# lifthrasiir/j40

Measured on AMD Instinct MI355X. Metric: Mpixels/s RGBA-u8x4 decode, 8K VarDCT d1, higher is better.
Workload: dtype f32

## Files before the change

### j40_amd/csrc/device/hf_lanes_dev.h

```cpp
#pragma once
#include "hf_dev.h"

namespace j40hip {

struct LaneTables {
	const J40_LDS uint8_t *ctx_map;
	const J40_LDS uint32_t *cluster_cfg;
	const J40_LDS uint64_t *alias;
	const J40_LDS int16_t *nnz_ctx2;
	const J40_LDS int8_t *freq_ctx2;
	const J40_LDS uint32_t *dct_info;
	int32_t log_alpha, log_bucket;
};

struct LaneFrame {
	int32_t nb_block_ctx, num_hf_presets, preset_bits, check_section_end;
	uint32_t single_declared_end;
	const J40_GLOBAL uint32_t *order_off;
};

struct LaneGlobals {
	const J40_GLOBAL uint8_t *codestream;
	const J40_GLOBAL uint32_t *group_blocks;
	J40_GLOBAL float *coeffs;
	J40_GLOBAL CoeffEvent *events;
	J40_GLOBAL uint32_t *block_events;
	const J40_GLOBAL uint16_t *pool_u16;
	uint32_t coeff_stride;
};

struct LaneBits {
	const J40_GLOBAL uint8_t *base;
	uint64_t bits;
	int32_t nbits;
	uint32_t pos;
	uint32_t ahead;
};

J40_DEV uint32_t lane_load32(const J40_GLOBAL uint8_t *base, uint32_t pos) { return *(const J40_GLOBAL uint32_t *) (base + pos); }

J40_DEV void lane_bits_init(LaneBits &b, const J40_GLOBAL uint8_t *base, uint32_t start_bit) {
	b.base = base;
	const uint32_t pos0 = (start_bit >> 3) & ~3u, skip = start_bit - 8u * pos0;
	b.bits = (uint64_t) (lane_load32(base, pos0) >> skip);
	b.nbits = 32 - (int32_t) skip;
	b.pos = pos0 + 4;
	b.ahead = lane_load32(base, b.pos);
}

J40_DEV void lane_bits_refill(LaneBits &b) {
	if (b.nbits <= 32) {
		b.bits |= (uint64_t) b.ahead << b.nbits;
		b.nbits += 32;
		b.pos += 4u;
		b.ahead = lane_load32(b.base, b.pos);
	}
}

J40_DEV uint32_t lane_bits_take(LaneBits &b, int32_t n) {
	const uint32_t v = (uint32_t) b.bits & ((1u << n) - 1u);
	b.bits >>= n; b.nbits -= n;
	return v;
}

J40_DEV uint32_t lane_bit_position(const LaneBits &b) { return 8u * b.pos - (uint32_t) b.nbits; }

template <bool STRAIGHT = false, bool STARTED = false, class AliasPtr>
J40_DEV int32_t lane_symbol_in_cluster(LaneBits &b, uint32_t &state, AliasPtr alias, int32_t log_alpha, int32_t log_bucket, uint32_t cl, uint32_t m, uint32_t end_bit, uint32_t *err) {
	if (!STRAIGHT && !STARTED && state == 0) {
		state = lane_bits_take(b, 16); state |= lane_bits_take(b, 16) << 16;
		lane_bits_refill(b);
	}
	const uint32_t idx = state & 0xfff, i = idx >> log_bucket, pos = idx & ((1u << log_bucket) - 1);
	const uint64_t e = alias[(cl << log_alpha) + i];
	const uint32_t elo = (uint32_t) e, ehi = (uint32_t) (e >> 32);
	const bool aliased = pos >= (elo & 0xff);
	const int32_t token = (int32_t) (aliased ? (elo >> 20) & 0xff : i);
	const uint32_t offset = aliased ? (elo >> 8) & 0xfff : 0;
	const uint32_t d = aliased ? (uint32_t) (e >> 28) & 0x1fff : (ehi >> 9) & 0x1fff;
	state = d * (state >> 12) + offset + pos;
	const bool renorm = state < (1u << 16);
	const uint32_t low = lane_bits_take(b, renorm ? 16 : 0);
	state = renorm ? (state << 16) | low : state;
	const bool short1 = lane_bit_position(b) > end_bit;
	const int32_t split_exp = (int32_t) (m & 15), split = 1 << split_exp;
	const bool big = token >= split;
	const int32_t mt = (int32_t) (m >> 12);
	const bool iovf = big && token > mt;
	const int32_t tok = iovf ? mt : token;
	const int32_t msb = (int32_t) ((m >> 4) & 15), lsb = (int32_t) ((m >> 8) & 15), in_token = msb + lsb;
	const int32_t midbits = big ? split_exp - in_token + ((tok - split) >> in_token) : 0;
	if (!STRAIGHT && midbits > b.nbits) lane_bits_refill(b);
	const int32_t mid = (int32_t) lane_bits_take(b, midbits);
	const bool short2 = lane_bit_position(b) > end_bit;
	const int32_t top = 1 << msb;
	const int32_t lo = tok & ((1 << lsb) - 1), hi = (tok >> lsb) & (top - 1);
	const int32_t value = ((top | hi) << (midbits + lsb)) | ((mid << lsb) | lo);
	*err = short1 ? (uint32_t) ERR_SHRT : iovf ? (uint32_t) ERR_IOVF : short2 ? (uint32_t) ERR_SHRT : 0u;
	return big ? value : token;
}
template <class Tables>
J40_DEV int32_t lane_symbol(LaneBits &b, uint32_t &state, const Tables &t, int32_t ctx, uint32_t end_bit, uint32_t *err) {
	const uint32_t cl = t.ctx_map[ctx];
	return lane_symbol_in_cluster(b, state, t.alias, t.log_alpha, t.log_bucket, cl, t.cluster_cfg[cl], end_bit, err);
}

typedef uint32_t LaneEventQuad __attribute__((vector_size(16)));

J40_DEV void lane_store_block_events(const LaneGlobals &G, uint32_t blk, uint32_t first, uint32_t n0, uint32_t n1, uint32_t n2) {
	J40_GLOBAL uint64_t *e = (J40_GLOBAL uint64_t *) (G.block_events + 4u * blk);
	e[0] = (uint64_t) first | ((uint64_t) n0 << 32); e[1] = (uint64_t) n1 | ((uint64_t) n2 << 32);
}

struct LaneSection {
	uint32_t start_bit, end_bit;
	uint32_t cell_base;
	uint32_t block_first; int32_t nblocks;
	uint32_t ev_first, ev_end;
};

#ifndef J40_LANE_NZ_PERIOD
#define J40_LANE_NZ_PERIOD 8
#endif
#ifndef J40_LANE_STRAIGHT_COEFFS
#define J40_LANE_STRAIGHT_COEFFS 1
#endif
#ifndef J40_LANE_REFILL_SELECTS
#define J40_LANE_REFILL_SELECTS 0
#endif
template <bool SCAN, class Source>
J40_DEV void decode_hf_sections_lane(const LaneFrame &f, const LaneTables &t, const LaneGlobals &G, Source &src, J40_LDS int8_t *cols, int32_t col_stride, int32_t pass, J40_LDS uint32_t *ring = nullptr, int32_t ring_stride = 0) {
	LaneSection S;
	S.start_bit = S.end_bit = S.cell_base = S.block_first = S.ev_first = S.ev_end = 0; S.nblocks = 0;
	LaneBits b;
	b.base = G.codestream; b.bits = 0; b.nbits = 0; b.pos = 0; b.ahead = 0;
	const int32_t nb_block_ctx = f.nb_block_ctx;
	uint32_t err = 0, end_bit = 0, cell64 = 0, block_first = 0;
	int32_t nblocks = 0, ctxoff = 0;
	bool have = false;
	int32_t k = 0, c_yxb = 0;
	bool in_coeffs = false, done = true;
	uint32_t state = 0;
	int32_t x8 = 0, y8 = 0, log_columns = 3, order_idx = 0, shift = 0, size = 64;
	uint32_t coeffoff = 0, coeff_at = 0, bctx3 = 0;
	int32_t c = 1, bctx = 0, nz = 0, i = 0, prev = 0, cctx = 0;
	const J40_GLOBAL uint16_t *order = nullptr;
	uint32_t ev_at = 0, ev_end = 0, chan_first = 0;
	uint32_t ev_flushed = 0;
	uint32_t blk_first = 0, blk_n0 = 0, blk_n1 = 0;
	uint32_t next0 = 0, next1 = 0;
	for (uint32_t turn = 0; ; ++turn) {
#if J40_LANE_EV_FLUSH
		if (SCAN && (turn % J40_LANE_EV_FLUSH) == 0) {
#ifdef __HIPCC__
			asm volatile("");
#endif
			if (ev_at - ev_flushed >= (uint32_t) J40_LANE_EV_FLUSH) {
			const J40_LDS uint32_t *r = ring + (int32_t) (ev_flushed % (uint32_t) HF_LANE_RING_SLOTS) * ring_stride;
			J40_GLOBAL uint32_t *dst = (J40_GLOBAL uint32_t *) G.events + ev_flushed;
#pragma unroll
			for (int32_t k4 = 0; k4 < J40_LANE_EV_FLUSH; k4 += 4) {
				LaneEventQuad q4;
				q4[0] = r[k4 * ring_stride]; q4[1] = r[(k4 + 1) * ring_stride]; q4[2] = r[(k4 + 2) * ring_stride]; q4[3] = r[(k4 + 3) * ring_stride];
				*(J40_GLOBAL LaneEventQuad *) (dst + k4) = q4;
			}
			ev_flushed += (uint32_t) J40_LANE_EV_FLUSH;
			}
		}
#endif
		if (SCAN && J40_LANE_STRAIGHT_COEFFS) {
			if (in_coeffs && !done && state != 0) {
				if (J40_LANE_REFILL_SELECTS) {
					const bool need = b.nbits <= 32;
					b.bits |= (uint64_t) (need ? b.ahead : 0u) << (need ? b.nbits : 0);
					b.nbits += need ? 32 : 0; b.pos += need ? 4u : 0u;
					b.ahead = lane_load32(b.base, b.pos);
				} else lane_bits_refill(b);
				const int32_t cctx_now = cctx + t.nnz_ctx2[(nz + (1 << shift) - 1) >> shift] + t.freq_ctx2[i >> shift] + prev;
				uint32_t e2;
				const uint32_t cl = t.ctx_map[cctx_now];
				const int32_t v = lane_symbol_in_cluster<false, true>(b, state, t.alias, t.log_alpha, t.log_bucket, cl, t.cluster_cfg[cl], end_bit, &e2);
				const bool nonzero = v != 0 && e2 == 0;
				const int32_t sv = unpack_signed_dev(v);
				const bool full = nonzero && (ev_at >= ev_end || !coeff_event_fits(sv));
				if (nonzero && !full) {
					if (J40_LANE_EV_FLUSH) ring[(int32_t) (ev_at % (uint32_t) HF_LANE_RING_SLOTS) * ring_stride] = coeff_event_pack((uint32_t) i, sv);
					else ((J40_GLOBAL uint32_t *) G.events)[ev_at] = coeff_event_pack((uint32_t) i, sv);
				}
				ev_at += nonzero && !full ? 1u : 0u;
				e2 = e2 ? e2 : full ? (uint32_t) ERR_EVOF : 0u;
				prev = v != 0;
				nz -= prev;
				++i;
				in_coeffs = nz != 0;
				e2 = e2 ? e2 : in_coeffs && i >= size ? (uint32_t) ERR_COEF : 0u;
				const bool next_channel = !in_coeffs && e2 == 0;
				c_yxb += next_channel ? 1 : 0;
				const bool next_block = next_channel && c_yxb == 3;
				c_yxb = next_block ? 0 : c_yxb;
				k += next_block ? 1 : 0;
				err = e2 ? e2 : err;
				done = e2 != 0 || (next_block && k >= nblocks);
			}
			if ((turn % J40_LANE_NZ_PERIOD) != 0) continue;
#ifdef __HIPCC__
			asm volatile("");
#endif
			if (in_coeffs && !done && state != 0) continue;
		}
		if (done) {
			if (have) {
				if (SCAN && J40_LANE_EV_FLUSH) for (; ev_flushed < ev_at; ++ev_flushed) ((J40_GLOBAL uint32_t *) G.events)[ev_flushed] = ring[(int32_t) (ev_flushed % (uint32_t) HF_LANE_RING_SLOTS) * ring_stride];
				if (SCAN && !err && nblocks > 0) lane_store_block_events(G, block_first + (uint32_t) nblocks - 1u, blk_first, blk_n0, blk_n1, ev_at - chan_first);
				if (!err) {
					if (state == 0) { lane_bits_refill(b); state = lane_bits_take(b, 16); state |= lane_bits_take(b, 16) << 16; if (lane_bit_position(b) > end_bit) err = ERR_SHRT; }
					if (!err && state != 0x130000) err = ERR_ANS;
				}
				if (!err && f.check_section_end) {
					const uint32_t at = lane_bit_position(b), padn = (0u - at) & 7u;
					if (padn > (uint32_t) b.nbits) lane_bits_refill(b);
					if (lane_bits_take(b, (int32_t) padn)) err = ERR_PAD0;
					else if (at + padn != 8u * f.single_declared_end) err = at + padn < 8u * f.single_declared_end ? (uint32_t) ERR_SHRT : (uint32_t) ERR_EXCS;
				}
				src.done(err, lane_bit_position(b));
			}
			have = src.next(S);
			if (!have) break;
			end_bit = S.end_bit; cell64 = S.cell_base * 64u; block_first = S.block_first; nblocks = S.nblocks;
			lane_bits_init(b, G.codestream, S.start_bit);
			lane_bits_refill(b);
			err = 0;
			const uint32_t preset = lane_bits_take(b, f.preset_bits);
			if (lane_bit_position(b) > end_bit) err = ERR_SHRT;
			else if ((int32_t) preset >= f.num_hf_presets) err = ERR_RNGE;
			ctxoff = 495 * nb_block_ctx * (int32_t) preset;
			k = 0; c_yxb = 0; in_coeffs = false; state = 0;
			ev_at = chan_first = blk_first = ev_flushed = S.ev_first; ev_end = S.ev_end; blk_n0 = blk_n1 = 0;
			done = nblocks == 0 || err != 0;
			if (done) continue;
			{ const J40_GLOBAL uint32_t *p = G.group_blocks + 2u * block_first; next0 = p[0]; next1 = p[1]; }
		}
		if (!in_coeffs && (turn % J40_LANE_NZ_PERIOD) != 0) continue;
		lane_bits_refill(b);
		int32_t ctx;
		if (!in_coeffs) {
			if (SCAN) {
				const uint32_t n = ev_at - chan_first;
				if (c_yxb == 1) blk_n0 = n; else if (c_yxb == 2) blk_n1 = n;
				else if (k > 0) lane_store_block_events(G, block_first + (uint32_t) k - 1u, blk_first, blk_n0, blk_n1, n);
				chan_first = ev_at;
			}
			if (c_yxb == 0) {
				const uint32_t w = next1;
				coeffoff = next0 & ~15u;
				blk_first = ev_at;
				if (k + 1 < nblocks) { const J40_GLOBAL uint32_t *p = G.group_blocks + 2u * (block_first + (uint32_t) k + 1u); next0 = p[0]; next1 = p[1]; }
				x8 = (int32_t) (w & 31); y8 = (int32_t) ((w >> 5) & 31); bctx3 = w >> 16;
				const uint32_t di = t.dct_info[(w >> 10) & 31];
				log_columns = (int32_t) ((di >> 8) & 255); order_idx = (int32_t) (di >> 16);
				shift = (int32_t) (di & 255) + log_columns - 6; size = 64 << shift;
			}
			c = c_yxb == 0 ? 1 : c_yxb == 1 ? 0 : 2;
			bctx = (int32_t) ((bctx3 >> (4 * c_yxb)) & 15);
			const J40_LDS int8_t *col = cols + (c * 32 + x8) * col_stride;
			const int32_t left = x8 > 0 ? col[-col_stride] : -1, topv = y8 > 0 ? col[0] : -1;
			const int32_t pnz = left < 0 ? (topv < 0 ? 32 : topv) : topv < 0 ? left : (left + topv + 1) >> 1;
			ctx = ctxoff + bctx + (pnz < 8 ? pnz : 4 + pnz / 2) * nb_block_ctx;
		} else {
			ctx = cctx + t.nnz_ctx2[(nz + (1 << shift) - 1) >> shift] + t.freq_ctx2[i >> shift] + prev;
		}
		uint32_t e2;
		const int32_t v = lane_symbol(b, state, t, ctx, end_bit, &e2);
		if (!in_coeffs) {
			nz = v;
			e2 = e2 ? e2 : nz > (63 << shift) ? (uint32_t) ERR_COEF : 0u;
			const int8_t qnz = (int8_t) ((nz + (1 << shift) - 1) >> shift);
			J40_LDS int8_t *col = cols + (c * 32 + x8) * col_stride;
			for (int32_t q = 0; q < (1 << (log_columns - 3)); ++q) col[q * col_stride] = qnz;
			cctx = ctxoff + 458 * bctx + 37 * nb_block_ctx;
			prev = nz <= (size >> 4);
			i = 1 << shift;
			if (!SCAN) {
				coeff_at = (uint32_t) c * G.coeff_stride + cell64 + coeffoff;
				order = G.pool_u16 + f.order_off[(pass * 13 + order_idx) * 3 + c];
			}
			in_coeffs = nz > 0;
		} else {
			const bool nonzero = v != 0 && e2 == 0;
			if (SCAN) {
// ... 46 lines not shown
```

### j40_amd/csrc/device/kernels.hip

```cpp
#include <hip/hip_runtime.h>
#include <hip/hip_ext.h>
#include <type_traits>
#include <cstring>
#include <cstdlib>
#include "hf_dev.h"
#include "hf_lanes_dev.h"
#include "idct_dev.h"
#include "vardct_dev.h"
#include "special8_dev.h"
#include "large_dev.h"
#include "k2_iter_dev.h"
#include "hf_uni_dev.h"
#include "restore_dev.h"
#include "kernels.h"

namespace j40hip {

__constant__ float c_half_secants[256];
__constant__ float c_afv_basis[256];
__device__ float c_srgb_thr[SRGB_TABLE_FLOATS];

#define J40_STAGE_SRGB_THRESHOLDS(f) \
	__shared__ float s_srgb_thr[SRGB_TABLE_FLOATS]; \
	for (int32_t i_ = threadIdx.x; i_ < SRGB_TABLE_FLOATS; i_ += blockDim.x) s_srgb_thr[i_] = c_srgb_thr[i_]; \
// ... 241 lines not shown
	const J40_GLOBAL DevPlan &plan = ((const J40_GLOBAL DevPlan *) plans)[w.frame];
	const J40_GLOBAL DevFrame &df = *(const J40_GLOBAL DevFrame *) plan.frame;
	const bool active = lane < w.num_groups;
	auto align16 = [](uint32_t v) { return (v + 15u) & ~15u; };
	LaneFrame f;
	f.nb_block_ctx = df.nb_block_ctx; f.num_hf_presets = df.num_hf_presets; f.preset_bits = df.preset_bits; f.check_section_end = df.check_section_end; f.single_declared_end = df.single_declared_end;
	f.order_off = df.order_off;
	const int32_t num_passes = df.num_passes, num_groups = df.num_groups, scan = df.sparse_coeffs;
	LaneGlobals G;
	G.codestream = (const J40_GLOBAL uint8_t *) plan.codestream;
	G.group_blocks = (const J40_GLOBAL uint32_t *) plan.group_blocks;
	G.coeffs = (J40_GLOBAL float *) plan.coeffs[0];
	G.events = (J40_GLOBAL CoeffEvent *) plan.events; G.block_events = (J40_GLOBAL uint32_t *) plan.block_events;
	G.pool_u16 = (const J40_GLOBAL uint16_t *) plan.pool_u16;
	G.coeff_stride = plan.coeff_stride;
	const J40_GLOBAL uint8_t *pool_u8 = (const J40_GLOBAL uint8_t *) plan.pool_u8;
	const J40_GLOBAL int32_t *pool_i32 = (const J40_GLOBAL int32_t *) plan.pool_i32;
	const J40_GLOBAL uint64_t *pool_u64 = (const J40_GLOBAL uint64_t *) plan.pool_u64;
	const J40_GLOBAL DevCodeSpec *specs = (const J40_GLOBAL DevCodeSpec *) plan.coeff_specs;
	const J40_GLOBAL DevCluster *clusters = (const J40_GLOBAL DevCluster *) plan.clusters;
	LaneQueue q;
	q.sections = (const J40_GLOBAL DevSection *) plan.sections; q.lf_groups = (const J40_GLOBAL DevLfGroup *) plan.lf_groups;
	q.block_start = (const J40_GLOBAL uint32_t *) plan.group_block_start; q.ev_range = (const J40_GLOBAL uint32_t *) plan.ev_range;
	q.lane_order = (const J40_GLOBAL uint32_t *) plan.lane_order;
	q.status = (J40_GLOBAL uint32_t *) plan.status; q.end_bits = df.sections_have_trailer ? (J40_GLOBAL uint32_t *) plan.section_end_bit : nullptr;
	q.counter = w.pad && queue && num_passes == 1 ? (J40_GLOBAL uint32_t *) queue + w.frame : nullptr;
	q.num_groups = num_groups; q.scan = scan != 0; q.g = 0;

	J40_LDS uint8_t *lds = (J40_LDS uint8_t *) hf_lds;
	J40_LDS int16_t *l_nnz = (J40_LDS int16_t *) lds;
	J40_LDS int8_t *l_freq = (J40_LDS int8_t *) (lds + 128);
	J40_LDS uint32_t *l_dct = (J40_LDS uint32_t *) (lds + 192);
	const uint32_t off_pass = 192 + 112;
	if (tid < 64) { l_nnz[tid] = DEV_NNZ_CTX2[tid]; l_freq[tid] = DEV_FREQ_CTX2[tid]; }
	if (tid < 27) l_dct[tid] = (uint32_t) DEV_DCT_SELECT[tid][0] | ((uint32_t) DEV_DCT_SELECT[tid][1] << 8) | ((uint32_t) DEV_DCT_SELECT[tid][2] << 16);
	LaneTables t;
	t.nnz_ctx2 = l_nnz; t.freq_ctx2 = l_freq; t.dct_info = l_dct;
	J40_LDS int8_t *l_cols = (J40_LDS int8_t *) (lds + lds_tables_bytes + (uint32_t) (tid >> 6) * HF_LANE_COLS_BYTES) + lane;
	J40_LDS uint32_t *l_ring = (J40_LDS uint32_t *) (lds + lds_tables_bytes + (uint32_t) (tid >> 6) * HF_LANE_COLS_BYTES + HF_LANE_PRED_BYTES) + lane;
	for (int32_t pass = 0; pass < num_passes; ++pass) {
		const J40_GLOBAL DevCodeSpec &spec = specs[pass];
		__syncthreads();
		const int32_t num_dist = spec.num_dist, num_clusters = spec.num_clusters, log_alpha = spec.log_alpha_size;
		J40_LDS uint8_t *l_map = lds + off_pass;
		J40_LDS uint32_t *l_cfg = (J40_LDS uint32_t *) (lds + off_pass + align16((uint32_t) num_dist));
		J40_LDS uint64_t *l_alias = (J40_LDS uint64_t *) ((J40_LDS uint8_t *) l_cfg + align16(4u * (uint32_t) num_clusters));
		{
			const J40_GLOBAL uint32_t *msrc = (const J40_GLOBAL uint32_t *) (pool_u8 + spec.cluster_map_off);
			J40_LDS uint32_t *mdst = (J40_LDS uint32_t *) l_map;
			for (int32_t i = tid; i < (num_dist + 3) / 4; i += blockDim.x) mdst[i] = msrc[i];
			const J40_GLOBAL int32_t *csrc = pool_i32 + spec.lane_cfg_off;
			for (int32_t i = tid; i < num_clusters; i += blockDim.x) l_cfg[i] = (uint32_t) csrc[i];
			const J40_GLOBAL uint64_t *asrc = pool_u64 + clusters[spec.cluster_off].table_off;
			for (uint32_t i = tid; i < ((uint32_t) num_clusters << log_alpha); i += blockDim.x) l_alias[i] = asrc[i];
		}
		t.ctx_map = l_map; t.cluster_cfg = l_cfg; t.alias = l_alias; t.log_alpha = log_alpha; t.log_bucket = 12 - log_alpha;
		__syncthreads();
		q.pass = pass; q.slot = active ? w.first_group + lane : -1;
		if (scan) decode_hf_sections_lane<true>(f, t, G, q, l_cols, 64, pass, l_ring, 64);
		else decode_hf_sections_lane<false>(f, t, G, q, l_cols, 64, pass);
	}
}

void launch_hf_lanes(const DevPlan *plans, const HfLaneWork *work, int32_t num_work, int32_t waves_per_wg, uint32_t lds_bytes, hipStream_t stream, hipEvent_t started, hipEvent_t stopped, uint32_t *queue) {
	if (num_work <= 0) return;
	static bool configured = false;
	if (!configured) { (void) hipFuncSetAttribute((const void *) k_hf_lanes, hipFuncAttributeMaxDynamicSharedMemorySize, 160 * 1024); configured = true; }
	const uint32_t tables = (lds_bytes + 15u) & ~15u;
	if (started && stopped) hipExtLaunchKernelGGL(k_hf_lanes, dim3((unsigned) (num_work / waves_per_wg)), dim3(64u * (unsigned) waves_per_wg), tables + (uint32_t) waves_per_wg * HF_LANE_COLS_BYTES, stream, started, stopped, 0, plans, work, tables, queue);
	else hipLaunchKernelGGL(k_hf_lanes, dim3((unsigned) (num_work / waves_per_wg)), dim3(64u * (unsigned) waves_per_wg), tables + (uint32_t) waves_per_wg * HF_LANE_COLS_BYTES, stream, plans, work, tables, queue);
}

uint32_t hf_lanes_lds_bytes(const HfLaunchInfo &info) {
	auto align16 = [](uint32_t v) { return (v + 15u) & ~15u; };
	uint32_t n = align16(info.block_ctx_size) + 192;
	if (info.tables_fit_lds) n += align16(info.max_num_dist) + align16(info.max_clusters * (uint32_t) sizeof(DevCluster)) + align16(info.max_table_bytes);
	return n;
}

void launch_hf_entropy_lanes(const DevPlan *plans, const HfLaneWork *work, int32_t num_work, bool tables_in_lds, uint32_t lds_bytes, hipStream_t stream) {
	if (num_work <= 0) return;
	if (tables_in_lds) {
		static bool configured = false;
		if (!configured) { (void) hipFuncSetAttribute((const void *) k_hf_entropy_lanes<true>, hipFuncAttributeMaxDynamicSharedMemorySize, 160 * 1024); configured = true; }
		hipLaunchKernelGGL(k_hf_entropy_lanes<true>, dim3((unsigned) num_work), dim3(64), lds_bytes, stream, plans, work);
	} else {
		hipLaunchKernelGGL(k_hf_entropy_lanes<false>, dim3((unsigned) num_work), dim3(64), lds_bytes, stream, plans, work);
	}
}


#ifdef J40_K2_PHASES
__device__ unsigned long long g_k2_phase[64][8];
#define K2_PHASES_BEGIN unsigned long long k2_acc[8] = {0, 0, 0, 0, 0, 0, 0, 0}; unsigned long long k2_last = __builtin_amdgcn_s_memtime()
#define K2_PHASE(i) do { const unsigned long long now_ = __builtin_amdgcn_s_memtime(); k2_acc[i] += now_ - k2_last; k2_last = now_; } while (0)
#define K2_PHASES_END(slot) do { if (threadIdx.x == 0) for (int i_ = 0; i_ < 8; ++i_) atomicAdd(&g_k2_phase[slot][i_], k2_acc[i_]); } while (0)
extern "C" __attribute__((visibility("default"))) void j40hip_debug_k2_phases(unsigned long long *out, int reset) {
	(void) hipDeviceSynchronize();
	(void) hipMemcpyFromSymbol(out, HIP_SYMBOL(g_k2_phase), sizeof(unsigned long long) * 64 * 8, 0, hipMemcpyDeviceToHost);
	if (reset) { static unsigned long long zero[64 * 8]; (void) hipMemcpyToSymbol(HIP_SYMBOL(g_k2_phase), zero, sizeof zero, 0, hipMemcpyHostToDevice); }
}
#else
#define K2_PHASES_BEGIN do { } while (0)
#define K2_PHASE(i) do { } while (0)
#define K2_PHASES_END(slot) do { } while (0)
#endif

__device__ __forceinline__ void uniform_plan(DevPlan &p) {
	p.frame = uni(p.frame); p.pool_u16 = uni(p.pool_u16); p.pool_f32 = uni(p.pool_f32); p.events = uni(p.events); p.block_events = uni(p.block_events);
	for (int c = 0; c < 3; ++c) { p.llf[c] = uni(p.llf[c]); p.coeffs[c] = uni(p.coeffs[c]); }
	p.coeff_stride = uni(p.coeff_stride);
}
// ... 776 lines not shown
```

### j40_amd/csrc/device/lf_rows_dev.h

```cpp
#pragma once
#include "lf_lanes_dev.h"
#include "modular_dev.h"

namespace j40hip {

enum { LF_USES_RAW = 1u << 8 };
J40_DEV uint32_t lf_stopped_at(int32_t chan, int32_t done) { return ((uint32_t) chan << 24) | (uint32_t) done; }

enum { LF_ROW_WIN = 256,
       LF_ROW_PITCH = LF_ROW_WIN + 2 };

struct LfRowTables {
	const J40_LDS DevTreeNode *tree;
	const J40_LDS uint32_t *fast;
	const J40_GLOBAL uint64_t *alias;
	int32_t log_alpha, log_bucket;
	uint32_t uses;
};

typedef uint32_t LfFastQuad __attribute__((vector_size(16)));
enum { LF_FAST_IOVF = 1u << 18, LF_FAST_IOVF_BASE = 1u << 30 };
J40_DEV void lf_rows_token_info(uint32_t tok, uint32_t cfg, uint32_t *base, uint32_t *extra, uint32_t *iovf) {
	const uint32_t split_exp = cfg & 15u, split = 1u << split_exp, msb = (cfg >> 4) & 15u, lsb = (cfg >> 8) & 15u, in_token = msb + lsb, mt = cfg >> 12;
	*base = tok; *extra = 0; *iovf = 0;
// ... 265 lines not shown
		return;
	}
	L.flush_n = ((cw - 1) & (LF_ROW_WIN - 1)) + 1; L.flush_dst = L.row + (cw - L.flush_n);
	L.x = 0; L.y = y + 1; L.row += cw; L.pw = L.pww = 0; L.a0 = L.a1 = 0;
	if (L.y < L.chh) {
		if (wide) { L.a2 = L.row[-cw]; L.a3 = L.row[1 - cw]; L.a4 = L.row[2 - cw]; }
		else { L.a2 = L.win[0]; L.a3 = cw > 1 ? L.win[1] : 0; L.a4 = cw > 2 ? L.win[2] : 0; }
		return;
	}
	++L.chan; L.setup = true;
}

J40_DEV int32_t lf_row_plain_run(const LfRowLane &L) {
	const bool can = L.plain_ok & !L.setup & (L.chan < 7) & (L.state != 0) & (!L.plain_wide | (L.x > 0));
	const int32_t last = L.plain_wide ? mod_min(L.cw - 1, L.x | (LF_ROW_WIN - 1)) : L.cw - 1;
	return can ? mod_max(last + 1 - L.x, 0) : 0;
}
J40_DEV void lf_row_run_end(LfRowLane &L) {
	if (lf_row_deferred(L)) return;
	const int32_t cw = L.cw, nx = L.x;
	if (nx < cw) {
		L.flush_n = LF_ROW_WIN; L.flush_dst = L.row + (nx - LF_ROW_WIN);
		return;
	}
	L.flush_n = ((cw - 1) & (LF_ROW_WIN - 1)) + 1; L.flush_dst = L.row + (cw - L.flush_n);
	L.x = 0; L.y += 1; L.row += cw; L.pw = L.pww = 0; L.a0 = L.a1 = 0;
	if (L.y < L.chh) {
		if (cw > LF_ROW_WIN) { L.a2 = L.row[-cw]; L.a3 = L.row[1 - cw]; L.a4 = L.row[2 - cw]; }
		else { L.a2 = L.win[0]; L.a3 = cw > 1 ? L.win[1] : 0; L.a4 = cw > 2 ? L.win[2] : 0; }
		return;
	}
	++L.chan; L.setup = true;
}
J40_DEV void lf_row_step(LfRowLane &L, const J40_GLOBAL DevLfTask &t, const LfRowTables &T) {
	if (L.in_run) lf_row_run_end(L); else lf_row_step_general(L, t, T);
	L.plain_left = lf_row_plain_run(L);
	L.in_run = L.plain_left > 0;
	L.live = !lf_row_done(L);
}

#ifdef __HIPCC__
J40_DEV int32_t lf_mad24(int32_t a, int32_t b, int32_t c) { int32_t d; asm("v_mad_i32_i24 %0, %1, %2, %3" : "=v"(d) : "v"(a), "v"(b), "v"(c)); return d; }
#else
J40_DEV int32_t lf_mad24(int32_t a, int32_t b, int32_t c) { return a * b + c; }
#endif
J40_DEV int32_t lf_unzigzag(int32_t u) { return (int32_t) ((uint32_t) u >> 1) ^ -(u & 1); }

enum { LF_NEED_TEST = 1,
       LF_NEED_LIN = 2, LF_NEED_SEL = 4, LF_NEED_GRAD = 8,
       LF_NEED_MUL = 16,
       LF_NEED_ALL = 31,
       LF_NEED_PRED = LF_NEED_TEST | LF_NEED_LIN | LF_NEED_SEL | LF_NEED_GRAD };

#ifdef __HIPCC__
J40_DEV uint32_t lf_bfe(uint32_t v, uint32_t off, uint32_t width) { return __builtin_amdgcn_ubfe(v, off, width); }
J40_DEV uint32_t lf_renorm_word(uint32_t state, uint32_t window) { return __builtin_amdgcn_perm(state, window, 0x05040100u); }
#else
J40_DEV uint32_t lf_bfe(uint32_t v, uint32_t off, uint32_t width) { return width ? (v >> off) & (0xffffffffu >> (32u - width)) : 0u; }
J40_DEV uint32_t lf_renorm_word(uint32_t state, uint32_t window) { return (state << 16) | (window & 0xffffu); }
#endif

template <uint32_t NEED>
J40_DEV void lf_row_step_plain_for(LfRowLane &L, const LfRowTables &T, J40_LDS int16_t *&wp) {
	LaneBits &b = L.b;
	{
		const bool need = b.nbits <= 32;
		const uint32_t inc = need ? 4u : 0u;
		b.bits |= (uint64_t) (need ? b.ahead : 0u) << (b.nbits & 63);
		b.nbits += (int32_t) (8u * inc); b.pos += inc;
		b.ahead = lane_load32(b.base, b.pos);
	}
	uint32_t word = L.k_word_le;
	int32_t pw = 0, pn = 0, pnw = 0, pne = 0, pww = 0, ahead3 = 0;
	if (NEED & LF_NEED_PRED) {
		const int32_t x = L.x, y = L.y, cw = L.cw;
		L.x = x + 1;
		ahead3 = wp[3];
		const bool up = y > 0, left = x > 0;
		pw = left ? L.pw : up ? L.a2 : 0;
		pn = up ? L.a2 : pw;
		pnw = left && up ? L.a1 : pw;
		pne = x + 1 < cw && up ? L.a3 : pn;
		pww = x > 1 ? L.pww : pw;
		if (NEED & LF_NEED_TEST) {
			const int32_t pnww = x > 1 && up ? L.a0 : pww;
			int32_t val = lf_mad24(L.c_x, x, lf_mad24(L.c_y, y, lf_mad24(L.c_w, pw, lf_mad24(L.c_n, pn, 0)))) + lf_mad24(L.c_nw, pnw, lf_mad24(L.c_ne, pne, lf_mad24(L.c_ww, pww, lf_mad24(L.c_nww, pnww, 0))));
			val = L.c_abs ? mod_abs(val) : val;
			val = L.c_first && !left ? pw : val;
			word = val > L.k_thr ? L.k_word_gt : L.k_word_le;
		}
	}
	const uint32_t st = L.state, bucket = lf_bfe(st, (uint32_t) T.log_bucket, (uint32_t) T.log_alpha), pos = st & ((1u << T.log_bucket) - 1u);
	const LfFastQuad e = *(const J40_LDS LfFastQuad *) (T.fast + 4u * ((word >> 24) << T.log_alpha) + 4u * bucket);
	const bool aliased = pos >= (e[0] & 0xffu);
	const uint32_t w = aliased ? e[1] : e[0] >> 8, base = aliased ? e[3] : e[2];
	const uint32_t state = (w & 0x1fffu) * (st >> 12) + (w >> 19) + pos;
	const bool renorm = state < (1u << 16);
	const uint32_t window = (uint32_t) b.bits, skip = renorm ? 16u : 0u, extra = (w >> 13) & 31u;
	L.state = renorm ? lf_renorm_word(state, window) : state;
	const uint32_t mid = lf_bfe(window, skip, extra), taken = skip + extra;
	b.bits >>= taken; b.nbits -= (int32_t) taken;
	const int32_t u = (int32_t) (base + (mid << ((word >> 8) & 15u)));
	int32_t pred = 0;
	if (NEED & LF_NEED_LIN) {
		int32_t lin = lf_mad24(L.p_w, pw, lf_mad24(L.p_n, pn, 0)) + lf_mad24(L.p_nw, pnw, lf_mad24(L.p_ne, pne, lf_mad24(L.p_ww, pww, 0)));
		pred = L.p_half ? (lin + (int32_t) ((uint32_t) lin >> 31)) >> 1 : lin;
	}
	if (NEED & LF_NEED_SEL) {
		const int32_t sel = mod_abs(pn - pnw) < mod_abs(pw - pnw) ? pw : pn;
		pred = (NEED & (LF_NEED_LIN | LF_NEED_GRAD)) ? (L.p_kind == 1 ? sel : pred) : sel;
	}
	if (NEED & LF_NEED_GRAD) {
		const int32_t grad = mod_gradient(pw, pn, pnw);
// ... 118 lines not shown
```

### j40_amd/csrc/device/plan.h

```cpp
#pragma once
#include <stdint.h>

namespace j40hip {

struct DevCluster {
	uint32_t cfg;
	int32_t max_token;
	uint32_t table_off;
	int16_t fast_len, max_len;
};

struct DevCodeSpec {
	int32_t num_dist, num_clusters;
	int32_t lz77_enabled, use_prefix_code;
	int32_t min_symbol, min_length;
	int32_t log_alpha_size;
	uint32_t lz_len_cfg;
	int32_t lz_len_max_token;
	uint32_t cluster_map_off;
	uint32_t cluster_off;
	uint32_t table_span;
	uint32_t lane_cfg_off;
};

struct DevLfGroup {
	int32_t left, top, width, height;
	int32_t width8, height8, width64, height64;
	int32_t cell_base;
	int32_t vb_base;
	int32_t c64_base;
	int32_t nb_varblocks;
	float mult_lf[3];
	int32_t pad;
};

struct DevSection {
	uint32_t byte_off, size, bit_off;
	int32_t ggidx;
	int32_t gx8, gy8;
	int32_t gw8, gh8;
	int32_t gx, gy, gw, gh;
};

struct DevGroupBlock {
	uint32_t coeffoff_qfidx;
	uint16_t pos_dct;
	uint16_t bctx3;
};

struct DevVarblock {
	int32_t coeff_base;
	int32_t llf_base;
	float mult1;
	float kx_hf;
	int32_t px, py;
	uint16_t effw, effh;
	uint8_t dctsel, pad[3];
	int32_t blk;
	float kb_hf;
};

struct DevFrame {
	int32_t width, height;
	int32_t num_passes, num_groups, num_lf_groups;
	int32_t nb_block_ctx, nb_qf_thr, lfidx_size, num_hf_presets, preset_bits;
	int32_t bpp;
	float quant_bias[3], quant_bias_num;
	float mult_base;
	float x_qm_mul, b_qm_mul;
	float kx_lf, kb_lf;
	float base_corr_x, base_corr_b, inv_colour_factor;
	float opsin_inv_mat[9], opsin_bias[3], cbrt_opsin_bias[3];
	float itscale;
	uint32_t order_off[11 * 13 * 3];
	uint32_t dq_off[17];
// ... 278 lines not shown
```

### j40_amd/csrc/plan_build.cpp

```cpp
#include "plan_build.hpp"
#include <algorithm>
#include <atomic>
#include <chrono>
#include <cmath>
#include <thread>

namespace j40hip {

namespace {
struct TeamBarrier {
	std::atomic<int> waiting{0}, generation{0}, team{1};
	void wait() {
		const int n = team.load(std::memory_order_acquire);
		if (n <= 1) return;
		const int g = generation.load(std::memory_order_acquire);
		if (waiting.fetch_add(1, std::memory_order_acq_rel) + 1 == n) { waiting.store(0, std::memory_order_relaxed); generation.fetch_add(1, std::memory_order_release); }
		else while (generation.load(std::memory_order_acquire) == g) std::this_thread::yield();
	}
};
template <class F> void run_team(int threads, F &body) {
	TeamBarrier bar;
	if (threads <= 1) { body(0, 1, bar); return; }
	std::vector<std::thread> pool;
	std::atomic<int> go{0};
	try {
		for (int t = 1; t < threads; ++t) pool.emplace_back([&, t] { int n; while ((n = go.load(std::memory_order_acquire)) == 0) std::this_thread::yield(); if (t < n) body(t, n, bar); });
	} catch (const std::exception &) { }
	const int n = (int) pool.size() + 1;
	bar.team.store(n, std::memory_order_release);
	go.store(n, std::memory_order_release);
	body(0, n, bar);
	for (std::thread &t : pool) t.join();
}
}

template <typename T> static uint32_t push(std::vector<T> &pool, const T *p, size_t n) { uint32_t off = (uint32_t) pool.size(); pool.insert(pool.end(), p, p + n); return off; }

void flatten_code_spec(const CodeSpec &spec, std::vector<uint8_t> &u8, std::vector<int32_t> &i32, std::vector<uint64_t> &u64, std::vector<DevCluster> &clusters, DevCodeSpec *out) {
	out->num_dist = spec.num_dist; out->num_clusters = spec.num_clusters;
	out->lz77_enabled = spec.lz77_enabled; out->use_prefix_code = spec.use_prefix_code;
	out->min_symbol = spec.min_symbol; out->min_length = spec.min_length;
	out->log_alpha_size = spec.log_alpha_size;
	out->lz_len_cfg = spec.lz_len_cfg.packed(); out->lz_len_max_token = spec.lz_len_cfg.max_token;
	while (u8.size() & 3) u8.push_back(0);
	out->cluster_map_off = push(u8, spec.cluster_map.data(), spec.cluster_map.size());
	while (u8.size() & 3) u8.push_back(0);
	out->cluster_off = (uint32_t) clusters.size();
	const size_t span0 = spec.use_prefix_code ? i32.size() : u64.size();
	for (const Cluster &c : spec.clusters) {
		DevCluster d;
		d.cfg = c.cfg.packed(); d.max_token = c.cfg.max_token;
		d.fast_len = (int16_t) c.fast_len; d.max_len = (int16_t) c.max_len;
		d.table_off = spec.use_prefix_code ? push(i32, c.table.data(), c.table.size()) : push(u64, c.alias.data(), c.alias.size());
		clusters.push_back(d);
	}
	out->table_span = (uint32_t) ((spec.use_prefix_code ? i32.size() : u64.size()) - span0);
	out->lane_cfg_off = 0xffffffffu;
	bool uniform = !spec.use_prefix_code && !spec.lz77_enabled && spec.num_clusters <= 256;
	for (const Cluster &c : spec.clusters) uniform = uniform && c.alias.size() == ((size_t) 1 << spec.log_alpha_size);
	if (uniform) {
		std::vector<int32_t> cfg;
		for (const Cluster &c : spec.clusters) cfg.push_back((int32_t) (c.cfg.packed() | ((uint32_t) std::min(c.cfg.max_token, 0xfffff) << 12)));
		out->lane_cfg_off = push(i32, cfg.data(), cfg.size());
	}
}

void fill_sections(const Frame &fr, std::vector<DevSection> *sections) {
	const int32_t num_groups = (int32_t) fr.fh.num_groups;
	sections->assign((size_t) fr.fh.num_passes * (size_t) num_groups, DevSection());
	for (int32_t p = 0; p < fr.fh.num_passes; ++p) for (int32_t g = 0; g < num_groups; ++g) {
		DevSection &d = (*sections)[(size_t) p * (size_t) num_groups + (size_t) g];
		const GroupInfo gi = group_info(fr.fh, g);
		if (fr.toc.single) {
			d.byte_off = (uint32_t) fr.toc.single_section.offset; d.size = (uint32_t) fr.toc.single_section.size; d.bit_off = (uint32_t) fr.single_pass_group_bitpos;
		} else {
			const Section &s0 = fr.toc.pass_groups[(size_t) p * (size_t) num_groups + (size_t) g];
			d.byte_off = (uint32_t) s0.offset; d.size = (uint32_t) s0.size; d.bit_off = 0;
		}
		d.ggidx = gi.ggidx; d.gx8 = gi.gx_in_gg / 8; d.gy8 = gi.gy_in_gg / 8;
		d.gw8 = ceil_div(gi.gw, 8); d.gh8 = ceil_div(gi.gh, 8);
		d.gx = fr.lf_groups[(size_t) gi.ggidx].left + gi.gx_in_gg; d.gy = fr.lf_groups[(size_t) gi.ggidx].top + gi.gy_in_gg; d.gw = gi.gw; d.gh = gi.gh;
	}
}

bool fill_event_ranges(const std::vector<DevSection> &sections, int32_t num_groups, bool sparse, std::vector<uint32_t> *ev_range, size_t *ev_capacity) {
	ev_range->clear(); *ev_capacity = 0;
	if (!sparse) return true;
	for (int32_t g = 0; g < num_groups; ++g) {
		const DevSection &d = sections[(size_t) g];
		static const size_t per_byte = getenv("J40HIP_EVENTS_PER_BYTE") ? (size_t) atoi(getenv("J40HIP_EVENTS_PER_BYTE")) : 4;
		const size_t worst = (size_t) d.gw8 * (size_t) d.gh8 * 64 * 3, cap = std::min(worst, (size_t) d.size * per_byte + 256);
		*ev_capacity = (*ev_capacity + 31) & ~(size_t) 31;
		ev_range->push_back((uint32_t) *ev_capacity);
		*ev_capacity += cap;
		ev_range->push_back((uint32_t) *ev_capacity);
	}
	if (*ev_capacity >= 0xffffffffull) { ev_range->clear(); *ev_capacity = 0; return false; }
	return true;
}

void fill_hf_launch_info(const std::vector<DevCodeSpec> &coeff_specs, uint32_t block_ctx_size, size_t coeff_floats, HfLaunchInfo *out) {
	HfLaunchInfo &hf = *out;
	hf.block_ctx_size = block_ctx_size; hf.max_num_dist = hf.max_clusters = hf.max_table_bytes = 0;
	for (const DevCodeSpec &sp : coeff_specs) {
		hf.max_num_dist = std::max<uint32_t>(hf.max_num_dist, (uint32_t) sp.num_dist);
		hf.max_clusters = std::max<uint32_t>(hf.max_clusters, (uint32_t) sp.num_clusters);
		hf.max_table_bytes = std::max<uint32_t>(hf.max_table_bytes, sp.table_span * (sp.use_prefix_code ? 4u : 8u));
	}
	{
		const uint32_t per_wave = 32 * 32 * 3 + 1024 * (uint32_t) sizeof(DevGroupBlock) + 16;
		const uint32_t fixed = hf.block_ctx_size + 256 + 64 + HF_WAVES * per_wave;
		hf.tables_fit_lds = fixed + hf.max_num_dist + hf.max_clusters * (uint32_t) sizeof(DevCluster) + hf.max_table_bytes + 64 <= 150u * 1024u;
	}
	{
		auto align16 = [](uint32_t v) { return (v + 15u) & ~15u; };
		hf.lanes_fast = true; hf.lanes_lds_bytes = 0;
		for (const DevCodeSpec &sp : coeff_specs) {
			hf.lanes_fast = hf.lanes_fast && sp.lane_cfg_off != 0xffffffffu;
			const uint32_t n = 128 + 64 + 112 + align16((uint32_t) sp.num_dist) + align16(4u * (uint32_t) sp.num_clusters) + 8u * ((uint32_t) sp.num_clusters << sp.log_alpha_size);
			hf.lanes_lds_bytes = std::max(hf.lanes_lds_bytes, n);
		}
		hf.lanes_fast = hf.lanes_fast && hf.lanes_lds_bytes + 4u * HF_LANE_COLS_BYTES <= 156u * 1024u && coeff_floats * 3 * sizeof(float) < 0xffffffffull;
	}
}

void fill_frame_constants(const Frame &fr, DevFrame *out) {
	DevFrame &df = *out;
	memset(&df, 0, sizeof df);
	df.width = fr.fh.width; df.height = fr.fh.height;
	df.num_passes = fr.fh.num_passes; df.num_groups = (int32_t) fr.fh.num_groups; df.num_lf_groups = (int32_t) fr.fh.num_lf_groups;
	df.nb_block_ctx = fr.nb_block_ctx; df.nb_qf_thr = fr.nb_qf_thr;
	df.lfidx_size = (fr.nb_lf_thr[0] + 1) * (fr.nb_lf_thr[1] + 1) * (fr.nb_lf_thr[2] + 1);
	df.num_hf_presets = fr.num_hf_presets; df.preset_bits = ceil_lg32((uint32_t) fr.num_hf_presets);
	df.bpp = fr.im.bpp;
	df.sections_have_trailer = (int32_t) fr.gmodular.channel.size() > fr.num_gm_channels;
	df.check_section_end = fr.toc.single && !df.sections_have_trailer;
	df.single_declared_end = (uint32_t) fr.toc.single_declared_end;
	for (int c = 0; c < 3; ++c) { df.quant_bias[c] = fr.im.quant_bias[c]; df.opsin_bias[c] = fr.im.opsin_bias[c]; df.cbrt_opsin_bias[c] = cbrtf(fr.im.opsin_bias[c]); }
	df.quant_bias_num = fr.im.quant_bias_num;
	static const float QM_SCALE[8] = {1.5625f, 1.25f, 1.0f, 0.8f, 0.64f, 0.512f, 0.4096f, 0.32768f};
	df.mult_base = 65536.0f / (float) fr.global_scale;
	df.x_qm_mul = QM_SCALE[fr.fh.x_qm_scale]; df.b_qm_mul = QM_SCALE[fr.fh.b_qm_scale];
	df.kx_lf = fr.base_corr_x + (float) fr.x_factor_lf * fr.inv_colour_factor;
	df.kb_lf = fr.base_corr_b + (float) fr.b_factor_lf * fr.inv_colour_factor;
	df.base_corr_x = fr.base_corr_x; df.base_corr_b = fr.base_corr_b; df.inv_colour_factor = fr.inv_colour_factor;
	for (int i = 0; i < 3; ++i) for (int j = 0; j < 3; ++j) df.opsin_inv_mat[i * 3 + j] = fr.im.opsin_inv_mat[i][j];
	df.itscale = 255.0f / fr.im.intensity_target;

}

uint32_t build_vardct_plan(const Frame &fr, const uint8_t *cs, size_t cs_size, HostPlan *hp, int threads) {
	static const bool timing = getenv("J40HIP_PLAN_TIMING") != nullptr;
	auto now = [] { return std::chrono::duration<double, std::milli>(std::chrono::steady_clock::now().time_since_epoch()).count(); };
	const double tb0 = timing ? now() : 0; double tbA = 0, tbB = 0, tbC = 0;
	if (cs_size + 16 >= ((size_t) 1 << 29)) return ERR_TODO;
	if (fr.fh.is_modular) return ERR_TODO;
	if (fr.im.grey || fr.fh.do_ycbcr) return ERR_TODO;
	if (fr.im.bpp < 8 || fr.im.exp_bits) return ERR_TODO;

	DevFrame &df = hp->frame;
	fill_frame_constants(fr, &df);
	hp->coeff_specs.assign((size_t) fr.fh.num_passes, DevCodeSpec());
	for (int32_t p = 0; p < fr.fh.num_passes; ++p) flatten_code_spec(fr.coeff_codespec[p], hp->pool_u8, hp->pool_i32, hp->pool_u64, hp->clusters, &hp->coeff_specs[(size_t) p]);
	hp->block_ctx_map_off = push(hp->pool_u8, fr.block_ctx_map.data(), fr.block_ctx_map.size());
	hp->pool_u8.resize(hp->pool_u8.size() + 16, 0);
	for (size_t i = 0; i < 11 * 13 * 3; ++i) df.order_off[i] = 0xffffffffu;
	for (int32_t p = 0; p < fr.fh.num_passes; ++p) for (int o = 0; o < 13; ++o) for (int c = 0; c < 3; ++c) {
		const std::vector<int32_t> &ord = fr.orders[p][o][c];
		if (ord.empty()) continue;
		std::vector<uint16_t> tmp(ord.size());
		for (size_t i = 0; i < ord.size(); ++i) tmp[i] = (uint16_t) ord[i];
		df.order_off[(p * 13 + o) * 3 + c] = push(hp->pool_u16, tmp.data(), tmp.size());
// ... 616 lines not shown
```

Baseline: 12770.

## Add fast HF lane symbol decode with precomputed token tables in LDS

```diff
diff --git a/j40_amd/csrc/device/hf_lanes_dev.h b/j40_amd/csrc/device/hf_lanes_dev.h
--- a/j40_amd/csrc/device/hf_lanes_dev.h
+++ b/j40_amd/csrc/device/hf_lanes_dev.h
@@ -11,6 +11,7 @@
 	const J40_LDS int8_t *freq_ctx2;
 	const J40_LDS uint32_t *dct_info;
 	int32_t log_alpha, log_bucket;
+	const J40_LDS uint64_t *tok;
 };
 
 struct LaneFrame {
@@ -105,6 +106,45 @@
 	return lane_symbol_in_cluster(b, state, t.alias, t.log_alpha, t.log_bucket, cl, t.cluster_cfg[cl], end_bit, err);
 }
 
+#ifdef __HIPCC__
+J40_DEV uint32_t lf_bfe(uint32_t v, uint32_t off, uint32_t width) { return __builtin_amdgcn_ubfe(v, off, width); }
+J40_DEV uint32_t lf_renorm_word(uint32_t state, uint32_t window) { return __builtin_amdgcn_perm(state, window, 0x05040100u); }
+#else
+J40_DEV uint32_t lf_bfe(uint32_t v, uint32_t off, uint32_t width) { return width ? (v >> off) & (0xffffffffu >> (32u - width)) : 0u; }
+J40_DEV uint32_t lf_renorm_word(uint32_t state, uint32_t window) { return (state << 16) | (window & 0xffffu); }
+#endif
+
+enum : uint32_t { LANE_TOK_DEFER = 1u << 31 };
+J40_DEV uint64_t lane_token_entry(uint32_t tok, uint32_t cfg) {
+	const uint32_t split_exp = cfg & 15u, split = 1u << split_exp, msb = (cfg >> 4) & 15u, lsb = (cfg >> 8) & 15u, in_token = msb + lsb, mt = cfg >> 12;
+	if (tok < split) return tok;
+	if (tok > mt) return (uint64_t) LANE_TOK_DEFER << 32;
+	const uint32_t midbits = split_exp - in_token + ((tok - split) >> in_token);
+	if (midbits > 16u) return (uint64_t) LANE_TOK_DEFER << 32;
+	const uint32_t top = 1u << msb, lo = tok & ((1u << lsb) - 1u), hi = (tok >> lsb) & (top - 1u);
+	return (uint64_t) (((top | hi) << (midbits + lsb)) | lo) | ((uint64_t) (midbits | (lsb << 8)) << 32);
+}
+
+template <class AliasPtr, class TokPtr>
+J40_DEV int32_t lane_symbol_fast(LaneBits &b, uint32_t &state, AliasPtr alias, TokPtr tok, int32_t log_alpha, int32_t log_bucket, uint32_t cl, uint32_t &defer) {
+	const uint32_t idx = state & 0xfff, i = idx >> log_bucket, pos = idx & ((1u << log_bucket) - 1);
+	const uint64_t e = alias[(cl << log_alpha) + i];
+	const uint32_t elo = (uint32_t) e, ehi = (uint32_t) (e >> 32);
+	const bool aliased = pos >= (elo & 0xff);
+	const uint32_t token = aliased ? (elo >> 20) & 0xff : i;
+	const uint32_t offset = aliased ? (elo >> 8) & 0xfff : 0;
+	const uint32_t d = aliased ? (uint32_t) (e >> 28) & 0x1fff : (ehi >> 9) & 0x1fff;
+	const uint64_t te = tok[((ehi >> 22) << log_alpha) + token];
+	const uint32_t st = d * (state >> 12) + offset + pos;
+	const bool renorm = st < (1u << 16);
+	const uint32_t window = (uint32_t) b.bits, skip = renorm ? 16u : 0u, thi = (uint32_t) (te >> 32), extra = thi & 31u;
+	state = renorm ? lf_renorm_word(st, window) : st;
+	const uint32_t mid = lf_bfe(window, skip, extra), taken = skip + extra;
+	b.bits >>= taken; b.nbits -= (int32_t) taken;
+	defer |= thi;
+	return (int32_t) ((uint32_t) te + (mid << ((thi >> 8) & 15u)));
+}
+
 typedef uint32_t LaneEventQuad __attribute__((vector_size(16)));
 
 J40_DEV void lane_store_block_events(const LaneGlobals &G, uint32_t blk, uint32_t first, uint32_t n0, uint32_t n1, uint32_t n2) {
@@ -128,8 +168,9 @@
 #ifndef J40_LANE_REFILL_SELECTS
 #define J40_LANE_REFILL_SELECTS 0
 #endif
-template <bool SCAN, class Source>
+template <bool SCAN, bool FAST = false, class Source>
 J40_DEV void decode_hf_sections_lane(const LaneFrame &f, const LaneTables &t, const LaneGlobals &G, Source &src, J40_LDS int8_t *cols, int32_t col_stride, int32_t pass, J40_LDS uint32_t *ring = nullptr, int32_t ring_stride = 0) {
+	static_assert(!FAST || SCAN, "the fast path is the sparse coefficients' straight path");
 	LaneSection S;
 	S.start_bit = S.end_bit = S.cell_base = S.block_first = S.ev_first = S.ev_end = 0; S.nblocks = 0;
 	LaneBits b;
@@ -149,6 +190,7 @@
 	uint32_t ev_flushed = 0;
 	uint32_t blk_first = 0, blk_n0 = 0, blk_n1 = 0;
 	uint32_t next0 = 0, next1 = 0;
+	uint32_t defer = 0, lim = 0;
 	for (uint32_t turn = 0; ; ++turn) {
 #if J40_LANE_EV_FLUSH
 		if (SCAN && (turn % J40_LANE_EV_FLUSH) == 0) {
@@ -169,7 +211,34 @@
 		}
 #endif
 		if (SCAN && J40_LANE_STRAIGHT_COEFFS) {
-			if (in_coeffs && !done && state != 0) {
+			if (FAST && in_coeffs && !done && state != 0) {
+				if (b.nbits <= 32) {
+					b.bits |= (uint64_t) b.ahead << b.nbits;
+					b.nbits += 32; b.pos += 4u;
+					b.ahead = lane_load32(b.base, b.pos < lim ? b.pos : lim);
+				}
+				const int32_t cctx_now = cctx + t.nnz_ctx2[(nz + (1 << shift) - 1) >> shift] + t.freq_ctx2[i >> shift] + prev;
+				const int32_t v = lane_symbol_fast(b, state, t.alias, t.tok, t.log_alpha, t.log_bucket, t.ctx_map[cctx_now], defer);
+				const bool nonzero = v != 0;
+				const int32_t sv = unpack_signed_dev(v);
+				const bool full = nonzero && (ev_at >= ev_end || !coeff_event_fits(sv));
+				if (nonzero && !full) {
+					if (J40_LANE_EV_FLUSH) ring[(int32_t) (ev_at % (uint32_t) HF_LANE_RING_SLOTS) * ring_stride] = coeff_event_pack((uint32_t) i, sv);
+					else ((J40_GLOBAL uint32_t *) G.events)[ev_at] = coeff_event_pack((uint32_t) i, sv);
+				}
+				ev_at += nonzero && !full ? 1u : 0u;
+				defer |= full ? (uint32_t) LANE_TOK_DEFER : 0u;
+				prev = nonzero;
+				nz -= prev;
+				++i;
+				in_coeffs = nz != 0 && i < size;
+				c_yxb += in_coeffs ? 0 : 1;
+				const bool next_block = !in_coeffs && c_yxb == 3;
+				c_yxb = next_block ? 0 : c_yxb;
+				k += next_block ? 1 : 0;
+				done = next_block && k >= nblocks;
+			} else
+			if (!FAST && in_coeffs && !done && state != 0) {
 				if (J40_LANE_REFILL_SELECTS) {
 					const bool need = b.nbits <= 32;
 					b.bits |= (uint64_t) (need ? b.ahead : 0u) << (need ? b.nbits : 0);
@@ -208,6 +277,7 @@
 #endif
 			if (in_coeffs && !done && state != 0) continue;
 		}
+		if (FAST && have && !err && (((defer & (uint32_t) LANE_TOK_DEFER) | (in_coeffs ? 0u : (uint32_t) nz)) != 0 || lane_bit_position(b) > end_bit)) { err = ERR_EVOF; done = true; }
 		if (done) {
 			if (have) {
 				if (SCAN && J40_LANE_EV_FLUSH) for (; ev_flushed < ev_at; ++ev_flushed) ((J40_GLOBAL uint32_t *) G.events)[ev_flushed] = ring[(int32_t) (ev_flushed % (uint32_t) HF_LANE_RING_SLOTS) * ring_stride];
@@ -235,6 +305,7 @@
 			else if ((int32_t) preset >= f.num_hf_presets) err = ERR_RNGE;
 			ctxoff = 495 * nb_block_ctx * (int32_t) preset;
 			k = 0; c_yxb = 0; in_coeffs = false; state = 0;
+			nz = 0; defer = 0; lim = ((end_bit >> 3) & ~3u) + 8u;
 			ev_at = chan_first = blk_first = ev_flushed = S.ev_first; ev_end = S.ev_end; blk_n0 = blk_n1 = 0;
 			done = nblocks == 0 || err != 0;
 			if (done) continue;
diff --git a/j40_amd/csrc/device/kernels.hip b/j40_amd/csrc/device/kernels.hip
--- a/j40_amd/csrc/device/kernels.hip
+++ b/j40_amd/csrc/device/kernels.hip
@@ -317,12 +317,16 @@
 			const J40_GLOBAL int32_t *csrc = pool_i32 + spec.lane_cfg_off;
 			for (int32_t i = tid; i < num_clusters; i += blockDim.x) l_cfg[i] = (uint32_t) csrc[i];
 			const J40_GLOBAL uint64_t *asrc = pool_u64 + clusters[spec.cluster_off].table_off;
-			for (uint32_t i = tid; i < ((uint32_t) num_clusters << log_alpha); i += blockDim.x) l_alias[i] = asrc[i];
+			const J40_GLOBAL int32_t *dsrc = pool_i32 + spec.lane_cfgs_off, *isrc = dsrc + spec.lane_num_cfgs;
+			for (uint32_t i = tid; i < ((uint32_t) num_clusters << log_alpha); i += blockDim.x) l_alias[i] = asrc[i] | ((uint64_t) isrc[i >> log_alpha] << 54);
+			J40_LDS uint64_t *l_tok = l_alias + ((uint32_t) num_clusters << log_alpha);
+			for (uint32_t i = tid; i < ((uint32_t) spec.lane_num_cfgs << log_alpha); i += blockDim.x) l_tok[i] = lane_token_entry(i & ((1u << log_alpha) - 1u), (uint32_t) dsrc[i >> log_alpha]);
+			t.tok = l_tok;
 		}
 		t.ctx_map = l_map; t.cluster_cfg = l_cfg; t.alias = l_alias; t.log_alpha = log_alpha; t.log_bucket = 12 - log_alpha;
 		__syncthreads();
 		q.pass = pass; q.slot = active ? w.first_group + lane : -1;
-		if (scan) decode_hf_sections_lane<true>(f, t, G, q, l_cols, 64, pass, l_ring, 64);
+		if (scan) decode_hf_sections_lane<true, true>(f, t, G, q, l_cols, 64, pass, l_ring, 64);
 		else decode_hf_sections_lane<false>(f, t, G, q, l_cols, 64, pass);
 	}
 }
diff --git a/j40_amd/csrc/device/lf_rows_dev.h b/j40_amd/csrc/device/lf_rows_dev.h
--- a/j40_amd/csrc/device/lf_rows_dev.h
+++ b/j40_amd/csrc/device/lf_rows_dev.h
@@ -341,13 +341,6 @@
        LF_NEED_ALL = 31,
        LF_NEED_PRED = LF_NEED_TEST | LF_NEED_LIN | LF_NEED_SEL | LF_NEED_GRAD };
 
-#ifdef __HIPCC__
-J40_DEV uint32_t lf_bfe(uint32_t v, uint32_t off, uint32_t width) { return __builtin_amdgcn_ubfe(v, off, width); }
-J40_DEV uint32_t lf_renorm_word(uint32_t state, uint32_t window) { return __builtin_amdgcn_perm(state, window, 0x05040100u); }
-#else
-J40_DEV uint32_t lf_bfe(uint32_t v, uint32_t off, uint32_t width) { return width ? (v >> off) & (0xffffffffu >> (32u - width)) : 0u; }
-J40_DEV uint32_t lf_renorm_word(uint32_t state, uint32_t window) { return (state << 16) | (window & 0xffffu); }
-#endif
 
 template <uint32_t NEED>
 J40_DEV void lf_row_step_plain_for(LfRowLane &L, const LfRowTables &T, J40_LDS int16_t *&wp) {
diff --git a/j40_amd/csrc/device/plan.h b/j40_amd/csrc/device/plan.h
--- a/j40_amd/csrc/device/plan.h
+++ b/j40_amd/csrc/device/plan.h
@@ -21,6 +21,8 @@
 	uint32_t cluster_off;
 	uint32_t table_span;
 	uint32_t lane_cfg_off;
+	uint32_t lane_cfgs_off;
+	int32_t lane_num_cfgs;
 };
 
 struct DevLfGroup {
diff --git a/j40_amd/csrc/plan_build.cpp b/j40_amd/csrc/plan_build.cpp
--- a/j40_amd/csrc/plan_build.cpp
+++ b/j40_amd/csrc/plan_build.cpp
@@ -55,13 +55,21 @@
 		clusters.push_back(d);
 	}
 	out->table_span = (uint32_t) ((spec.use_prefix_code ? i32.size() : u64.size()) - span0);
-	out->lane_cfg_off = 0xffffffffu;
+	out->lane_cfg_off = out->lane_cfgs_off = 0xffffffffu; out->lane_num_cfgs = 0;
 	bool uniform = !spec.use_prefix_code && !spec.lz77_enabled && spec.num_clusters <= 256;
 	for (const Cluster &c : spec.clusters) uniform = uniform && c.alias.size() == ((size_t) 1 << spec.log_alpha_size);
 	if (uniform) {
-		std::vector<int32_t> cfg;
+		std::vector<int32_t> cfg, distinct, index;
 		for (const Cluster &c : spec.clusters) cfg.push_back((int32_t) (c.cfg.packed() | ((uint32_t) std::min(c.cfg.max_token, 0xfffff) << 12)));
 		out->lane_cfg_off = push(i32, cfg.data(), cfg.size());
+		for (int32_t w : cfg) {
+			const size_t at = (size_t) (std::find(distinct.begin(), distinct.end(), w) - distinct.begin());
+			if (at == distinct.size()) distinct.push_back(w);
+			index.push_back((int32_t) at);
+		}
+		out->lane_num_cfgs = (int32_t) distinct.size();
+		out->lane_cfgs_off = push(i32, distinct.data(), distinct.size());
+		push(i32, index.data(), index.size());
 	}
 }
 
@@ -117,7 +125,8 @@
 		hf.lanes_fast = true; hf.lanes_lds_bytes = 0;
 		for (const DevCodeSpec &sp : coeff_specs) {
 			hf.lanes_fast = hf.lanes_fast && sp.lane_cfg_off != 0xffffffffu;
-			const uint32_t n = 128 + 64 + 112 + align16((uint32_t) sp.num_dist) + align16(4u * (uint32_t) sp.num_clusters) + 8u * ((uint32_t) sp.num_clusters << sp.log_alpha_size);
+			const uint32_t n = 128 + 64 + 112 + align16((uint32_t) sp.num_dist) + align16(4u * (uint32_t) sp.num_clusters) + 8u * ((uint32_t) sp.num_clusters << sp.log_alpha_size)
+				+ 8u * ((uint32_t) sp.lane_num_cfgs << sp.log_alpha_size);
 			hf.lanes_lds_bytes = std::max(hf.lanes_lds_bytes, n);
 		}
 		hf.lanes_fast = hf.lanes_fast && hf.lanes_lds_bytes + 4u * HF_LANE_COLS_BYTES <= 156u * 1024u && coeff_floats * 3 * sizeof(float) < 0xffffffffull;
```

Result: no change. 12630 (median of 2 runs) (-1.1%).
